# Sawyerbatch/simglucose

Measured on AMD Instinct MI355X. Metric: env-steps/sec at batch=1M patients (1-min dt); fp64 glucose trace max-abs-err, higher is better.
Workload: dtype f64

## Files before the change

simglucose_amd/csrc/t1d_abi.hip:

```cpp
#include "../../include/t1d.h"
#include "t1d_kernels.hpp"
#include "t1d_dopri5.hpp"
#include "t1d_policy.hpp"

#include <climits>
#include <cmath>
#include <cstdio>
#include <cstring>
#include <new>
#include <string>
#include <vector>

using namespace t1d;

struct t1d_ctx {
    int device = -1;
    int np = 0, S = 0;
    double sensor[T1D_SENSOR_NCOLS];
    double pump[T1D_PUMP_NCOLS];
    double* d_par64 = nullptr; float* d_par32 = nullptr;
    double* d_raw64 = nullptr;
    double* d_x0 = nullptr;
    double* d_minv64 = nullptr; float* d_minv32 = nullptr;
    int* d_status = nullptr;
    int math = 1;
    int n_cu = 256;
    int lds_per_block = 65536;
    std::vector<std::pair<const void*, size_t>> lds_allowed;
    int s1_blocks = 0;
    int split_refill = 1;
    int adaptive_gut = 1;
    int single_minute_kernel = 1;
    int integrator = -1;
    int split_nsub = 0;
    int np_pad = 0;
    double* d_prop64 = nullptr; float* d_prop32 = nullptr;
    long long* d_trace = nullptr;
    int defer_min_chunks = 1;
    int multi_minute_kernel = 1;
    int multi_minute_min_envs = 262144, multi_minute_min_envs_f32 = 393216;
    int park_cap = 0;
    int pingpong = 1;
    mutable unsigned launches = 0;
    int record_group_min = 64;
    int rollout_launches = 1;
    int rollout_launches_min_envs = 524288, rollout_launches_min_envs_f32 = 786432;
    int restart_compact = 1;
    std::vector<double> ptab;
    std::vector<double> dpar;
};

static thread_local std::string g_err;
static int fail(int code, const std::string& msg) { g_err = msg; return code; }
#define T1D_HIP(call)                                                                         \
    do {                                                                                      \
        hipError_t _e = (call);                                                               \
        if (_e != hipSuccess)                                                                 \
            return fail(T1D_E_HIP, std::string(#call) + ": " + hipGetErrorString(_e));        \
    } while (0)

static std::vector<double> spline_second_derivative_operator()
{
    const int K = 11;
    const double h = 15.0;
    std::vector<double> A(K * K, 0.0), B(K * K, 0.0);
    for (int k = 1; k < K - 1; ++k) {
        A[k * K + k - 1] = 1.0; A[k * K + k] = 4.0; A[k * K + k + 1] = 1.0;
        B[k * K + k - 1] = 6.0 / (h * h); B[k * K + k] = -12.0 / (h * h); B[k * K + k + 1] = 6.0 / (h * h);
    }
    A[0] = 1.0; A[1] = -2.0; A[2] = 1.0;
    A[(K - 1) * K + K - 3] = 1.0; A[(K - 1) * K + K - 2] = -2.0; A[(K - 1) * K + K - 1] = 1.0;
    for (int c = 0; c < K; ++c) {
        int piv = c;
        for (int r = c + 1; r < K; ++r) if (std::fabs(A[r * K + c]) > std::fabs(A[piv * K + c])) piv = r;
        if (piv != c) for (int j = 0; j < K; ++j) { std::swap(A[c * K + j], A[piv * K + j]); std::swap(B[c * K + j], B[piv * K + j]); }
        const double d = A[c * K + c];
        for (int j = 0; j < K; ++j) { A[c * K + j] /= d; B[c * K + j] /= d; }
        for (int r = 0; r < K; ++r) {
            if (r == c) continue;
            const double f = A[r * K + c];
            if (f == 0.0) continue;
            for (int j = 0; j < K; ++j) { A[r * K + j] -= f * A[c * K + j]; B[r * K + j] -= f * B[c * K + j]; }
        }
    }
    return B;
}


static void mat_expm(int n, const double* A, double* E)
{
    double nrm = 0.0;
    for (int i = 0; i < n; ++i) { double r = 0.0; for (int j = 0; j < n; ++j) r += std::fabs(A[i * n + j]); nrm = std::max(nrm, r); }
    int sq = 0;
    while (nrm > 0.03125 && sq < 60) { nrm *= 0.5; ++sq; }
    const double sc = std::ldexp(1.0, -sq);
    std::vector<double> B(n * n), term(n * n, 0.0), tmp(n * n);
    for (int k = 0; k < n * n; ++k) B[k] = A[k] * sc;
    for (int i = 0; i < n; ++i) { for (int j = 0; j < n; ++j) E[i * n + j] = (i == j); term[i * n + i] = 1.0; }
    for (int d = 1; d <= 16; ++d) {
        for (int i = 0; i < n; ++i)
            for (int j = 0; j < n; ++j) {
                double v = 0.0;
                for (int k = 0; k < n; ++k) v += term[i * n + k] * B[k * n + j];
                tmp[i * n + j] = v / (double)d;
            }
        term = tmp;
        for (int k = 0; k < n * n; ++k) E[k] += term[k];
    }
    for (int q = 0; q < sq; ++q) {
        for (int i = 0; i < n; ++i)
            for (int j = 0; j < n; ++j) {
                double v = 0.0;
                for (int k = 0; k < n; ++k) v += E[i * n + k] * E[k * n + j];
                tmp[i * n + j] = v;
            }
        for (int k = 0; k < n * n; ++k) E[k] = tmp[k];
    }
}

// ... 9 lines not shown
    at(5, 5) = -r[T1D_P_KI]; at(5, 0) = r[T1D_P_KI] / r[T1D_P_VI];
    at(6, 6) = -r[T1D_P_KI]; at(6, 5) = r[T1D_P_KI];
    double Ah[81], Ph[81], Pk[81], tmp[81];
    const int nb = 2 * n_sub;
    const double hb = 1.0 / (double)nb;
    for (int k = 0; k < 81; ++k) Ah[k] = A[k] * hb;
    mat_expm(9, Ah, Ph);
    std::memcpy(Pk, Ph, sizeof(Pk));
    static const int c6[7] = {4, 0, 1, 2, 3, 7, 8};
    static const int c8[7] = {6, 5, 0, 1, 2, 3, 7};
    for (int k = 1; k <= nb; ++k) {
        double* o = out + (k - 1) * 14;
        for (int j = 0; j < 7; ++j) { o[j] = Pk[4 * 9 + c6[j]]; o[7 + j] = Pk[6 * 9 + c8[j]]; }
        if (k == nb) break;
        for (int i = 0; i < 9; ++i)
            for (int j = 0; j < 9; ++j) {
                double v = 0.0;
                for (int q = 0; q < 9; ++q) v += Ph[i * 9 + q] * Pk[q * 9 + j];
                tmp[i * 9 + j] = v;
            }
        std::memcpy(Pk, tmp, sizeof(Pk));
    }
    double* t = out + 14 * nb;
    static const int c5[5] = {0, 1, 2, 3, 7};
    for (int j = 0; j < 5; ++j) { t[j] = Pk[0 * 9 + c5[j]]; t[5 + j] = Pk[1 * 9 + c5[j]]; }
    t[10] = Pk[2 * 9 + 2]; t[11] = Pk[2 * 9 + 7];
    t[12] = Pk[3 * 9 + 2]; t[13] = Pk[3 * 9 + 3]; t[14] = Pk[3 * 9 + 7];
    static const int c7[6] = {5, 0, 1, 2, 3, 7};
    for (int j = 0; j < 6; ++j) t[15 + j] = Pk[5 * 9 + c7[j]];
    const double h1 = 1.0 / (double)n_sub;
    const double hs[2] = {h1, 0.5 * h1};
    for (int part = 0; part < 2; ++part) {
        const double hh = hs[part], z = r[T1D_P_KABS] * hh;
        double I[3];
        for (int k = 0; k < 3; ++k) {
            double term = 1.0, sum = 0.0;
            for (int q = 1; q <= k + 1; ++q) term /= (double)q;
            for (int q = 1; q <= k; ++q) term *= (double)q;
            for (int j = 0; j < 60; ++j) {
                sum += term;
                term *= -z / (double)(k + j + 2);
                if (std::fabs(term) < 1e-30) break;
            }
            I[k] = sum;
        }
        double* w = out + kPropRows(n_sub) + 4 * part;
        w[0] = std::exp(-z);
        w[1] = hh * (2.0 * I[2] - 3.0 * I[1] + I[0]);
        w[2] = hh * (-4.0 * I[2] + 4.0 * I[1]);
        w[3] = hh * (2.0 * I[2] - I[1]);
    }
}

extern "C" int t1d_split_tables(const double* patient_row, int n_cols, int n_sub, double* out, int out_len)
{
    if (!patient_row || !out) return fail(T1D_E_INVALID, "t1d_split_tables: NULL argument");
    if (n_cols != T1D_P_NCOLS) return fail(T1D_E_INVALID, "t1d_split_tables: n_cols must be T1D_P_NCOLS (45)");
    if (n_sub < 2 || n_sub > 8 || (n_sub & 1)) return fail(T1D_E_INVALID, "t1d_split_tables: n_sub must be 2, 4, 6 or 8");
    if (out_len < kPropRows(n_sub) + 8) return fail(T1D_E_INVALID, "t1d_split_tables: out_len < 28 n_sub + 29");
    split_tables_row(patient_row, n_sub, out);
    return T1D_OK;
}

static int ensure_split(t1d_ctx* c, int ng)
{
    static_assert(DP_X2WB2 == DP_X2E + 7 && DP_X2E2 == DP_X2E + 4, "x2 weight rows are consecutive");
    if (c->split_nsub == ng) return T1D_OK;
    T1D_HIP(hipDeviceSynchronize());
    const int rows = kPropRows(ng), npp = c->np_pad;
    std::vector<double> prop((size_t)rows * npp, 0.0), one((size_t)rows + 8);
    for (int j = 0; j < c->np; ++j) {
        split_tables_row(c->ptab.data() + (size_t)j * T1D_P_NCOLS, ng, one.data());
        for (int k = 0; k < rows; ++k) prop[(size_t)k * npp + j] = one[k];
        for (int k = 0; k < 8; ++k) c->dpar[(size_t)(DP_X2E + k) * kMaxPatients + j] = one[rows + k];
    }
    std::vector<float> propf(prop.begin(), prop.end()), dpf(c->dpar.begin(), c->dpar.end());
    (void)hipFree(c->d_prop64); (void)hipFree(c->d_prop32); c->d_prop64 = nullptr; c->d_prop32 = nullptr;
    T1D_HIP(hipMalloc((void**)&c->d_prop64, prop.size() * 8));
    T1D_HIP(hipMalloc((void**)&c->d_prop32, propf.size() * 4));
    T1D_HIP(hipMemcpy(c->d_prop64, prop.data(), prop.size() * 8, hipMemcpyHostToDevice));
    T1D_HIP(hipMemcpy(c->d_prop32, propf.data(), propf.size() * 4, hipMemcpyHostToDevice));
    T1D_HIP(hipMemcpy(c->d_par64, c->dpar.data(), c->dpar.size() * 8, hipMemcpyHostToDevice));
    T1D_HIP(hipMemcpy(c->d_par32, dpf.data(), dpf.size() * 4, hipMemcpyHostToDevice));
    c->split_nsub = ng;
    return T1D_OK;
}

#if T1D_S1_TRACE
extern "C" int t1d_debug_trace(t1d_ctx* c, long long* out) { return hipMemcpy(out, c->d_trace, 128 * 4 * 64 * sizeof(long long), hipMemcpyDeviceToHost) == hipSuccess ? 0 : -1; }
#endif
extern "C" int t1d_abi_version(void) { return T1D_ABI_VERSION; }
extern "C" const char* t1d_last_error(void) { return g_err.c_str(); }

extern "C" int t1d_ctx_create(int hip_device, const double* ptab, int n_patients, int n_cols,
                              const double* sensor_row, const double* pump_row, t1d_ctx** out)
{
    try {
        if (!out) return fail(T1D_E_INVALID, "t1d_ctx_create: out is NULL");
        *out = nullptr;
        if (!ptab || !sensor_row || !pump_row) return fail(T1D_E_INVALID, "t1d_ctx_create: NULL table");
        if (n_cols != T1D_P_NCOLS) return fail(T1D_E_INVALID, "t1d_ctx_create: n_cols must be T1D_P_NCOLS (45)");
        if (n_patients < 1 || n_patients > kMaxPatients)
            return fail(T1D_E_INVALID, "t1d_ctx_create: n_patients must be in [1, 64]");
        const double st = sensor_row[5];
        if (!(st >= 1.0) || st != std::floor(st) || st > 1440.0)
            return fail(T1D_E_INVALID, "t1d_ctx_create: sensor sample_time must be a whole number of minutes >= 1");
        if (st > 150.0) return fail(T1D_E_INVALID, "t1d_ctx_create: sensor sample_time must be <= 150 minutes");
        for (int k = 2; k < 6; k += 3)
            if (!(pump_row[k] > 0.0)) return fail(T1D_E_INVALID, "t1d_ctx_create: pump increments must be > 0");
        int ndev = 0;
        if (hipGetDeviceCount(&ndev) != hipSuccess || ndev < 1)
            return fail(T1D_E_NODEVICE, "t1d_ctx_create: no HIP device visible");
        if (hip_device < 0 || hip_device >= ndev) return fail(T1D_E_INVALID, "t1d_ctx_create: bad device index");
        T1D_HIP(hipSetDevice(hip_device));
        int n_cu = 0;
        T1D_HIP(hipDeviceGetAttribute(&n_cu, hipDeviceAttributeMultiprocessorCount, hip_device));

        t1d_ctx* c = new (std::nothrow) t1d_ctx();
        if (!c) return fail(T1D_E_INVALID, "t1d_ctx_create: out of host memory");
        int lds_max = 0;
        if (hipDeviceGetAttribute(&lds_max, hipDeviceAttributeMaxSharedMemoryPerBlock, hip_device) == hipSuccess && lds_max > 0) c->lds_per_block = lds_max;
        c->device = hip_device; c->n_cu = n_cu > 0 ? n_cu : 256; c->np = n_patients; c->S = (int)std::floor(150.0 / st);
        std::memcpy(c->sensor, sensor_row, sizeof(c->sensor));
        std::memcpy(c->pump, pump_row, sizeof(c->pump));

        const int np = n_patients;
        std::vector<double> dp((size_t)DP_COUNT * kMaxPatients, 0.0), x0((size_t)13 * np);
        for (int j = 0; j < np; ++j) {
            const double* r = ptab + (size_t)j * n_cols;
            auto set = [&](int idx, double v) { dp[(size_t)idx * kMaxPatients + j] = v; };
            set(DP_KMAX, r[T1D_P_KMAX]); set(DP_KMIN, r[T1D_P_KMIN]); set(DP_KABS, r[T1D_P_KABS]);
            set(DP_HK, (r[T1D_P_KMAX] - r[T1D_P_KMIN]) / 2.0);
            set(DP_B, r[T1D_P_B]); set(DP_D, r[T1D_P_D]);
            set(DP_CAA, 5.0 / 2.0 / (1.0 - r[T1D_P_B])); set(DP_CCC, 5.0 / 2.0 / r[T1D_P_D]);
            set(DP_RATC, r[T1D_P_F] * r[T1D_P_KABS] / r[T1D_P_BW]);
            set(DP_KP1, r[T1D_P_KP1]); set(DP_KP2, r[T1D_P_KP2]); set(DP_KP3, r[T1D_P_KP3]);
            set(DP_FSNC, r[T1D_P_FSNC]); set(DP_KE1, r[T1D_P_KE1]); set(DP_KE2, r[T1D_P_KE2]);
            set(DP_K1, r[T1D_P_K1]); set(DP_K2, r[T1D_P_K2]); set(DP_VM0, r[T1D_P_VM0]);
            set(DP_VMX, r[T1D_P_VMX]); set(DP_KM0, r[T1D_P_KM0]);
            set(DP_M24, r[T1D_P_M2] + r[T1D_P_M4]); set(DP_M1, r[T1D_P_M1]);
            set(DP_KA1, r[T1D_P_KA1]); set(DP_KA2, r[T1D_P_KA2]); set(DP_VI, r[T1D_P_VI]);
            set(DP_P2U, r[T1D_P_P2U]); set(DP_IB, r[T1D_P_IB]); set(DP_KI, r[T1D_P_KI]);
            set(DP_M130, r[T1D_P_M1] + r[T1D_P_M30]); set(DP_M2, r[T1D_P_M2]);
            set(DP_KA1KD, r[T1D_P_KA1] + r[T1D_P_KD]); set(DP_KD, r[T1D_P_KD]); set(DP_KSC, r[T1D_P_KSC]);
            set(DP_INSC, 6000.0 / r[T1D_P_BW]); set(DP_VG, r[T1D_P_VG]); set(DP_IVI, 1.0 / r[T1D_P_VI]); set(DP_IVG, 1.0 / r[T1D_P_VG]);
            set(DP_DK, r[T1D_P_KMAX] - r[T1D_P_KMIN]);
            set(DP_CF, r[T1D_P_F] / r[T1D_P_BW]);
            for (int k = 0; k < 13; ++k) x0[(size_t)k * np + j] = r[T1D_P_X0 + k];
        }
        std::vector<double> raw((size_t)kRawPars * kMaxPatients, 0.0);
        for (int j = 0; j < np; ++j)
            for (int k = 0; k < kRawPars; ++k) raw[(size_t)k * kMaxPatients + j] = ptab[(size_t)j * n_cols + T1D_P_BW + k];
        c->ptab.assign(ptab, ptab + (size_t)np * n_cols);
        c->dpar = dp;
        c->np_pad = (np + 1) & ~1;
        std::vector<float> dpf(dp.begin(), dp.end());
        const std::vector<double> minv = spline_second_derivative_operator();
        std::vector<float> minvf(minv.begin(), minv.end());
        auto up = [&](void** dst, const void* src, size_t bytes) -> hipError_t {
            hipError_t e = hipMalloc(dst, bytes);
            if (e != hipSuccess) return e;
            return hipMemcpy(*dst, src, bytes, hipMemcpyHostToDevice);
        };
        hipError_t e = hipSuccess;
        if (e == hipSuccess) e = up((void**)&c->d_par64, dp.data(), dp.size() * 8);
        if (e == hipSuccess) e = up((void**)&c->d_par32, dpf.data(), dpf.size() * 4);
        if (e == hipSuccess) e = up((void**)&c->d_x0, x0.data(), x0.size() * 8);
        if (e == hipSuccess) e = up((void**)&c->d_raw64, raw.data(), raw.size() * 8);
        if (e == hipSuccess) e = up((void**)&c->d_minv64, minv.data(), minv.size() * 8);
        if (e == hipSuccess) e = up((void**)&c->d_minv32, minvf.data(), minvf.size() * 4);
#if T1D_S1_TRACE
        if (e == hipSuccess) e = hipMalloc((void**)&c->d_trace, 128 * 4 * 64 * sizeof(long long));
        if (e == hipSuccess) e = hipMemset(c->d_trace, 0, 128 * 4 * 64 * sizeof(long long));
#endif
        if (e == hipSuccess) e = hipMalloc((void**)&c->d_status, sizeof(int));
        if (e == hipSuccess) e = hipMemset(c->d_status, 0, sizeof(int));
        if (e != hipSuccess) {
            std::string m = std::string("t1d_ctx_create: ") + hipGetErrorString(e);
            t1d_ctx_destroy(c);
            return fail(T1D_E_HIP, m);
        }
        *out = c;
        return T1D_OK;
    } catch (const std::exception& ex) {
        return fail(T1D_E_INVALID, std::string("t1d_ctx_create: ") + ex.what());
    } catch (...) {
        return fail(T1D_E_INVALID, "t1d_ctx_create: unknown exception");
    }
}

extern "C" int t1d_ctx_set_option(t1d_ctx* c, const char* name, int64_t value)
{
    if (!c || !name) return fail(T1D_E_INVALID, "t1d_ctx_set_option: NULL argument");
    struct Opt { const char* name; int t1d_ctx::*field; int64_t lo, hi; };
    static const Opt opts[] = {
        {"math", &t1d_ctx::math, 0, 1},
        {"split_refill", &t1d_ctx::split_refill, 0, 1},
        {"defer_min_chunks", &t1d_ctx::defer_min_chunks, 0, 65535},
        {"multi_minute_kernel", &t1d_ctx::multi_minute_kernel, 0, 2},
        {"multi_minute_min_envs", &t1d_ctx::multi_minute_min_envs, 0, 1 << 28},
        {"multi_minute_min_envs_f32", &t1d_ctx::multi_minute_min_envs_f32, 0, 1 << 28},
        {"park_cap", &t1d_ctx::park_cap, 0, 65535},
        {"pingpong", &t1d_ctx::pingpong, 0, 1},
        {"record_group_min", &t1d_ctx::record_group_min, 1, 64},
        {"rollout_launches", &t1d_ctx::rollout_launches, 0, 2},
        {"rollout_launches_min_envs", &t1d_ctx::rollout_launches_min_envs, 0, 1 << 28},
        {"rollout_launches_min_envs_f32", &t1d_ctx::rollout_launches_min_envs_f32, 0, 1 << 28},
        {"restart_compact", &t1d_ctx::restart_compact, 0, 1},
        {"s1_blocks", &t1d_ctx::s1_blocks, 0, 65535},
        {"adaptive_gut", &t1d_ctx::adaptive_gut, 0, 3},
        {"single_minute_kernel", &t1d_ctx::single_minute_kernel, 0, 1},
        {"integrator", &t1d_ctx::integrator, -1, 1},
    };
    for (const Opt& o : opts)
        if (std::strcmp(name, o.name) == 0) {
            if (value < o.lo || value > o.hi)
                return fail(T1D_E_INVALID, std::string("t1d_ctx_set_option: ") + name + " must be in [" + std::to_string(o.lo) + ", " + std::to_string(o.hi) + "]");
            c->*(o.field) = (int)value;
            return T1D_OK;
        }
    return fail(T1D_E_INVALID, std::string("t1d_ctx_set_option: unknown option ") + name);
}

extern "C" int t1d_ctx_destroy(t1d_ctx* c)
{
    if (!c) return T1D_OK;
    (void)hipSetDevice(c->device);
    (void)hipFree(c->d_par64); (void)hipFree(c->d_par32); (void)hipFree(c->d_x0);
    (void)hipFree(c->d_minv64); (void)hipFree(c->d_minv32); (void)hipFree(c->d_status);
    (void)hipFree(c->d_prop64); (void)hipFree(c->d_prop32); (void)hipFree(c->d_trace); (void)hipFree(c->d_raw64);
    delete c;
    return T1D_OK;
}

static int check_batch(const char* who, const t1d_ctx* c, const t1d_batch* b, bool need_action)
{
    if (!c) return fail(T1D_E_INVALID, std::string(who) + ": ctx is NULL");
    if (!b) return fail(T1D_E_INVALID, std::string(who) + ": batch is NULL");
    if (b->n < 1 || b->n > (int64_t)1 << 28)
        return fail(T1D_E_INVALID, std::string(who) + ": batch.n out of range");
    if (b->dtype != T1D_F64 && b->dtype != T1D_F32) return fail(T1D_E_INVALID, std::string(who) + ": bad dtype");
    if (!b->x || !b->planned || !b->last_qsto || !b->last_food || !b->t || !b->meta || !b->last_cgm ||
        !b->ar_e || !b->pts || !b->prev_risk)
        return fail(T1D_E_INVALID, std::string(who) + ": a state pointer is NULL");
    if (!b->cgm || !b->bg || !b->reward || !b->done)
        return fail(T1D_E_INVALID, std::string(who) + ": cgm/bg/reward/done outputs are required");
    if (need_action && !b->basal) return fail(T1D_E_INVALID, std::string(who) + ": basal is NULL");
    if (b->n_meals < 0 || b->n_meals > 65535) return fail(T1D_E_INVALID, std::string(who) + ": n_meals out of range");
    if (b->n_meals > 0 && (!b->meal_time || !b->meal_amt))
        return fail(T1D_E_INVALID, std::string(who) + ": n_meals > 0 but meal table pointer is NULL");
    if (b->n_normals < 0) return fail(T1D_E_INVALID, std::string(who) + ": n_normals < 0");
    if (b->n_normals > 0 && !b->normals) return fail(T1D_E_INVALID, std::string(who) + ": n_normals > 0 but normals is NULL");
    const int known = T1D_BATCH_NO_PUMP | T1D_BATCH_NO_REFILL_DUE | (T1D_AB_FLAGS ? 0x1f00 : 0);
    if (b->flags & ~known) return fail(T1D_E_INVALID, std::string(who) + ": unknown bit in batch.flags");
    if (hipSetDevice(c->device) != hipSuccess) return fail(T1D_E_HIP, std::string(who) + ": hipSetDevice failed");
    return T1D_OK;
}

template <typename T>
static KArgs<T> make_args(const t1d_ctx* c, const t1d_batch* b, int minutes, int n_sub)
{
    KArgs<T> a;
    a.n = b->n; a.env_offset = b->env_offset; a.seed = b->seed;
    a.x = (T*)b->x; a.planned = (T*)b->planned; a.last_qsto = (T*)b->last_qsto; a.last_food = (T*)b->last_food;
    a.t = b->t; a.meta = b->meta; a.episode = b->episode; a.next_meal = b->next_meal;
    a.last_cgm = (T*)b->last_cgm; a.ar_e = (T*)b->ar_e; a.pts = (T*)b->pts; a.prev_risk = (T*)b->prev_risk; a.dbar = (T*)b->dbar;
    a.basal = (const T*)b->basal; a.bolus = (const T*)b->bolus; a.cho = (const T*)b->cho;
    a.meal_time = b->meal_time; a.meal_amt = (const T*)b->meal_amt;
    a.normals = b->n_normals > 0 ? (const T*)b->normals : nullptr;
    a.x0_override = (const T*)b->x0_override;
    a.cgm = (T*)b->cgm; a.bg = (T*)b->bg; a.reward = (T*)b->reward; a.done = b->done;
    a.lbgi = (T*)b->lbgi; a.hbgi = (T*)b->hbgi; a.risk = (T*)b->risk; a.meal = (T*)b->meal; a.insulin = (T*)b->insulin; a.cgm0 = (T*)b->cgm0;
    a.dpar = sizeof(T) == 8 ? (const T*)c->d_par64 : (const T*)c->d_par32;
    a.x0tab = c->d_x0;
    a.minv = sizeof(T) == 8 ? (const T*)c->d_minv64 : (const T*)c->d_minv32;
    a.status = c->d_status; a.trace = c->d_trace;
    a.sen.pacf = (T)c->sensor[0]; a.sen.gamma = (T)c->sensor[1]; a.sen.lambda = (T)c->sensor[2];
    a.sen.delta = (T)c->sensor[3]; a.sen.xi = (T)c->sensor[4]; a.sen.st = (int)c->sensor[5];
    a.sen.vmin = (T)c->sensor[6]; a.sen.vmax = (T)c->sensor[7];
    a.pump.min_bolus = (T)c->pump[0]; a.pump.max_bolus = (T)c->pump[1]; a.pump.inc_bolus = (T)c->pump[2];
    a.pump.min_basal = (T)c->pump[3]; a.pump.max_basal = (T)c->pump[4]; a.pump.inc_basal = (T)c->pump[5];
    a.np = c->np; a.S = c->S; a.n_meals = b->n_meals; a.n_normals = b->n_normals;
    a.minutes = minutes; a.n_sub = n_sub; a.flags = b->flags | (c->pingpong && (c->launches & 1) ? kFlagReverse : 0);
    a.prop = sizeof(T) == 8 ? (const T*)c->d_prop64 : (const T*)c->d_prop32;
    a.prop_rows = c->split_nsub ? kPropRows(c->split_nsub) : 0; a.np_pad = c->np_pad;
    return a;
}

static inline dim3 grid_for(int64_t n) { return dim3((unsigned)((n + kBlock - 1) / kBlock)); }

extern "C" int t1d_reset(t1d_ctx* c, const t1d_batch* b, const uint8_t* mask, int random_init_bg, void* stream)
{
    int rc = check_batch("t1d_reset", c, b, false);
    if (rc) return rc;
    hipStream_t s = (hipStream_t)stream;
    if (b->dtype == T1D_F64)
        hipLaunchKernelGGL(reset_kernel<double>, grid_for(b->n), dim3(kBlock), 0, s, make_args<double>(c, b, 1, 1), mask, random_init_bg);
    else
        hipLaunchKernelGGL(reset_kernel<float>, grid_for(b->n), dim3(kBlock), 0, s, make_args<float>(c, b, 1, 1), mask, random_init_bg);
    T1D_HIP(hipGetLastError());
    return T1D_OK;
}

static hipError_t allow_lds(t1d_ctx* c, const void* fn, size_t bytes)
{
    if (bytes <= 65536) return hipSuccess;
    for (auto& f : c->lds_allowed)
        if (f.first == fn) {
            if (f.second >= bytes) return hipSuccess;
            hipError_t e = hipFuncSetAttribute(fn, hipFuncAttributeMaxDynamicSharedMemorySize, (int)bytes);
            if (e == hipSuccess) f.second = bytes;
            return e;
        }
    hipError_t e = hipFuncSetAttribute(fn, hipFuncAttributeMaxDynamicSharedMemorySize, (int)bytes);
    if (e == hipSuccess) c->lds_allowed.push_back({fn, bytes});
    return e;
}

enum class Kern { step, rollout, step1, step1d, stepn };

struct Plan {
    Kern kernel = Kern::step;
    bool f64 = true;
    int variant = 0;
    bool refill = false;
    int stride = 32;
    bool extra = false;
    bool tiered = false;
    bool ctrl = false;
    bool refill_ahead = false;
    bool tables = false;
    unsigned grid = 0, block = 0;
    size_t lds = 0;
    int nchunks = 0, cap = 0, mode = 0;
};

static bool is_packed(const t1d_batch* b, size_t esz)
{
    const char* xb = (const char*)b->x;
    const size_t rowb = (size_t)b->n * esz;
    return (const char*)b->planned == xb + 13 * rowb && (const char*)b->last_qsto == xb + 14 * rowb &&
           (const char*)b->last_food == xb + 15 * rowb && (const char*)b->last_cgm == xb + 16 * rowb &&
           (const char*)b->prev_risk == xb + 17 * rowb && (const char*)b->pts == xb + 18 * rowb &&
           (const char*)b->dbar == xb + (size_t)kRowDbar * rowb &&
           b->next_meal && (const char*)b->meta == (const char*)b->t + (size_t)b->n * 4 &&
           (const char*)b->next_meal == (const char*)b->t + (size_t)b->n * 8 &&
           (size_t)kPackedRows * rowb < ((size_t)1 << 32);
}

static int plan_call(const char* who, const t1d_ctx* c, const t1d_batch* b, int minutes, int n_sub, bool rollout, Plan* out,
                     bool one_launch = false)
{
    Plan& p = *out;
    p = Plan();
    if (minutes < 1 || minutes > 100000) return fail(T1D_E_INVALID, std::string(who) + ": minutes out of range");
    if (n_sub < 1 || n_sub > 4096) return fail(T1D_E_INVALID, std::string(who) + ": n_sub out of range");
    bool split = c->math != 0 && n_sub >= 2 && n_sub <= 8 && !(n_sub & 1);
    if (c->integrator == 1 && !split)
        return fail(T1D_E_INVALID, std::string(who) + ": the split integrator needs math = 1 and n_sub in {2, 4, 6, 8}");
    split = split && c->integrator != 0;
    p.tables = split;
    p.f64 = b->dtype == T1D_F64;
    const size_t esz = p.f64 ? 8 : 4;
    p.extra = b->lbgi || b->hbgi || b->risk || b->meal || b->insulin;
    const bool split_refill = c->math != 0 && c->split_refill && minutes <= (int)c->sensor[5];

    const int stride = c->np <= 32 ? 32 : 64;
// ... 519 lines not shown
```

simglucose_amd/csrc/t1d_device.hpp:

```cpp
#pragma once
#include <hip/hip_runtime.h>
#include <rocrand/rocrand_kernel.h>
#include <stdint.h>

namespace t1d {

enum DevPar : int {
    DP_KMAX = 0, DP_KMIN, DP_KABS, DP_HK , DP_B, DP_D, DP_CAA ,
    DP_CCC , DP_RATC , DP_KP1, DP_KP2, DP_KP3, DP_FSNC, DP_KE1, DP_KE2,
    DP_K1, DP_K2, DP_VM0, DP_VMX, DP_KM0, DP_M24 , DP_M1, DP_KA1, DP_KA2, DP_VI, DP_P2U,
    DP_IB, DP_KI, DP_M130 , DP_M2, DP_KA1KD , DP_KD, DP_KSC, DP_INSC ,
    DP_VG, DP_IVI , DP_IVG , DP_DK ,
    DP_CF , DP_X2E , DP_X2WA, DP_X2WM, DP_X2WB,
    DP_X2E2, DP_X2WA2, DP_X2WM2, DP_X2WB2, DP_COUNT
};
constexpr int DP_RK4_COUNT = DP_CF;
constexpr int kMaxPatients = 64;
constexpr int kBlock = 256;

template <typename T> struct ParsLds {
    static constexpr bool kSplitRk4 = false;
    const T* base;
    int pid;
    __device__ __forceinline__ T operator()(int idx) const { return base[idx * kMaxPatients + pid]; }
// ... 496 lines not shown
__device__ __forceinline__ void rk4_minute(P& p, const MinuteIn<T>& u, T (&x)[13], int n_sub)
{
    if (MATH == 1 && P::kSplitRk4) {
        rk4_substeps_split(p, u, x, n_sub);
    } else {
        rk4_substeps<MATH>(p, u, x, n_sub);
    }
}

template <int MATH, typename T, typename P>
__device__ __forceinline__ void rk4_substeps(P& p, const MinuteIn<T>& u, T (&x)[13], int n_sub)
{
    const T h = T(1) / T(n_sub);
    const T hh = T(0.5) * h, h6 = h / T(6);
    T k[13], y[13], acc[13];
    for (int s = 0; s < n_sub; ++s) {
        rhs<MATH>(p, u, x, k);
#pragma unroll
        for (int i = 0; i < 13; ++i) { acc[i] = k[i]; y[i] = x[i] + hh * k[i]; }
        rhs<MATH>(p, u, y, k);
#pragma unroll
        for (int i = 0; i < 13; ++i) { acc[i] += T(2) * k[i]; y[i] = x[i] + hh * k[i]; }
        rhs<MATH>(p, u, y, k);
#pragma unroll
        for (int i = 0; i < 13; ++i) { acc[i] += T(2) * k[i]; y[i] = x[i] + h * k[i]; }
        rhs<MATH>(p, u, y, k);
#pragma unroll
        for (int i = 0; i < 13; ++i) x[i] = x[i] + h6 * (acc[i] + k[i]);
    }
}

__device__ __forceinline__ double dbar_of(double lq, double lf) { return fma(lf, 1000.0, lq); }
__device__ __forceinline__ float dbar_of(float lq, float lf) { return fmaf(lf, 1000.0f, lq); }

template <int MATH, typename T, typename P>
__device__ __forceinline__ MinuteIn<T> eat_minute(P& p, const T (&x)[13], T meal, T insulin_upm,
                                                  T& planned, T& last_qsto, T& last_food, bool& was_eating)
{
    T to_eat = T(0);
    planned += meal;
    if (planned > T(0)) {
        to_eat = planned < T(5) ? planned : T(5);
        planned -= to_eat;
        planned = planned > T(0) ? planned : T(0);
    }
    if (to_eat > T(0) && !was_eating) {
        last_qsto = x[0] + x[1];
        last_food = T(0);
    }
    last_food += to_eat;
    was_eating = to_eat > T(0);
    MinuteIn<T> u;
    u.d_mg = to_eat * T(1000);
    u.ins = insulin_upm * p(DP_INSC);
    const T dbar = dbar_of(last_qsto, last_food);
    u.has_dbar = dbar > T(0);
    const T dsafe = u.has_dbar ? dbar : T(1);
    if (MATH == 0) {
        u.aa = u.has_dbar ? p(DP_CAA) / dsafe : T(0);
        u.cc = u.has_dbar ? p(DP_CCC) / dsafe : T(0);
    } else {
        const T inv2 = u.has_dbar ? fdiv(T(2), dsafe) : T(0);
        u.aa = p(DP_CAA) * inv2;
        u.cc = p(DP_CCC) * inv2;
    }
    u.bD = p(DP_B) * dsafe;
    u.dD = p(DP_D) * dsafe;
    u.aabD = u.aa * u.bD;
    u.ccdD = u.cc * u.dD;
    return u;
}

template <typename T>
__device__ __forceinline__ T pump_quantise(T amount, T inc, T lo, T hi)
{
    T v = amount * T(6000);
    v = t_rint(v / inc) * inc;
    v = fdiv(v, T(6000));
    v = v < hi ? v : hi;
    v = v > lo ? v : lo;
    return v;
}

template <int MATH, typename T>
__device__ __forceinline__ void risk_index1(T bg, T& lbgi, T& hbgi, T& ri)
{
    T f;
    if (MATH == 0) {
        f = T(1.509) * (t_pow(t_log(bg), T(1.084)) - T(5.381));
    } else {
        const T inf = T(__builtin_huge_val());
        const T nan = T(__builtin_nan(""));
        const bool regular = bg > T(1) && bg < inf;
        const T u = log_core<true>(regular ? bg : T(2));
        const T pw = exp_core<12, true>(T(1.084) * log_core<true>(u));
        const T freg = T(1.509) * (pw - T(5.381));
        const T fodd = bg == T(1) ? T(1.509) * (T(0) - T(5.381)) : ((bg == T(0) || bg == inf) ? inf : nan);
        f = regular ? freg : fodd;
    }
    T l = T(0), h = T(0);
    const T ff = T(10) * f * f;
    l = f < T(0) ? ff : T(0);
    h = f > T(0) ? ff : T(0);
    const T big = sizeof(T) == 8 ? T(1.7976931348623157e308) : T(3.4028234663852886e38);
    l = l < big ? l : big;
    h = h < big ? h : big;
    lbgi = l; hbgi = h; ri = l + h;
}

template <typename T> struct SensorC { T pacf, gamma, lambda, delta, xi, vmin, vmax; int st; };
template <typename T> struct PumpC { T min_bolus, max_bolus, inc_bolus, min_basal, max_basal, inc_basal; };

template <bool FAST, typename T>
__device__ __forceinline__ T johnson_su(const SensorC<T>& s, T e)
{
    const T v = (e - s.gamma) / s.delta;
    if (!FAST) return s.xi + s.lambda * t_sinh(v);
    const T lim = sizeof(T) == 8 ? T(350) : T(40);
    const T E = exp_core(t_max(t_min(v, lim), -lim));
    return s.xi + s.lambda * (T(0.5) * (E - fdiv(T(1), E)));
}

__device__ __forceinline__ double2 philox_pair(uint64_t seed, uint64_t gid, uint32_t episode, uint32_t pair)
{
    rocrand_state_philox4x32_10 st;
    const unsigned long long off = 4ull * (((unsigned long long)episode << 24) + pair);
    rocrand_init(seed, gid, off, &st);
    return rocrand_normal_double2(&st);
}

}
```

simglucose_amd/csrc/t1d_kernels.hpp:

```cpp
#pragma once
#include "../../include/t1d.h"
#include "t1d_device.hpp"

#ifndef T1D_WAVES
#define T1D_WAVES 2
#endif
#ifndef T1D_ROW_RECOMPUTE
#define T1D_ROW_RECOMPUTE 1
#endif
constexpr int kFlagReverse = 0x10000;
#ifndef T1D_AB_FLAGS
#define T1D_AB_FLAGS 0
#endif

#include <climits>
#include <cstdint>
#include <type_traits>

namespace t1d {

template <typename T> struct KArgs {
    int64_t n, env_offset;
    uint64_t seed;
    T* x; T* planned; T* last_qsto; T* last_food; int32_t* t; uint32_t* meta; uint32_t* episode; int32_t* next_meal;
    T* last_cgm; T* ar_e; T* pts; T* prev_risk; T* dbar;
    const T* basal; const T* bolus; const T* cho; const int32_t* meal_time; const T* meal_amt;
    const T* normals; const T* x0_override;
    T* cgm; T* bg; T* reward; uint8_t* done; T* lbgi; T* hbgi; T* risk; T* meal; T* insulin; T* cgm0;
    const T* dpar;
    const T* prop;
    const double* x0tab;
    const T* minv;
    int* status;
    long long* trace;
    SensorC<T> sen; PumpC<T> pump;
    int np, S, n_meals, n_normals, minutes, n_sub, flags, prop_rows, np_pad;
};

template <typename T> struct PidArgs {
    T P, I, D, target;
    T* integ; T* prev; T* sum_risk; T* min_bg; T* max_bg; int32_t* n_low; int32_t* n_high;
    int n_steps;
    int kind;
    const T* bb_basal; const T* bb_cr; const T* bb_cf; T* bb_prev_meal;
    T* bg_trace; T* cgm_trace; T* cho_trace; T* ins_trace; int64_t trace_row;
};

template <typename U> __device__ __forceinline__ U* row(U* base, int64_t n, int k)
{
#if T1D_ROW_RECOMPUTE
    int kk = k;
    asm volatile("" : "+s"(kk));
    return base + (int64_t)kk * n;
#else
    U* p = base + (int64_t)k * n;
    asm volatile("" : "+s"(p));
    return p;
#endif
}
template <typename U> __device__ __forceinline__ U* rowv(U* base, int64_t n, int k) { return base + (int64_t)k * n; }
template <typename A> __device__ __forceinline__ bool ab_flag(const A& a, int bit) { return T1D_AB_FLAGS && (a.flags & bit) != 0; }
template <typename U> struct GRef {
    __attribute__((address_space(1))) U* p;
    __device__ __forceinline__ operator U() const { return *p; }
    __device__ __forceinline__ const GRef& operator=(U v) const { *p = v; return *this; }
};
template <typename U> __device__ __forceinline__ GRef<U> at(U* base, unsigned i)
{
    typedef __attribute__((address_space(1))) char gchar;
    typedef __attribute__((address_space(1))) U gU;
    return GRef<U>{(gU*)((gchar*)base + (unsigned)(i * (unsigned)sizeof(U)))};
}

typedef unsigned int t1d_v2u32 __attribute__((ext_vector_type(2)));
template <typename U> struct BRow { __amdgpu_buffer_rsrc_t r; int soff; };
template <typename U> struct BRef {
    __amdgpu_buffer_rsrc_t r; unsigned voff; int soff;
    __device__ __forceinline__ operator U() const
    {
        if constexpr (sizeof(U) == 8) return __builtin_bit_cast(U, __builtin_amdgcn_raw_buffer_load_b64(r, voff, soff, 0));
        else return __builtin_bit_cast(U, __builtin_amdgcn_raw_buffer_load_b32(r, voff, soff, 0));
    }
    __device__ __forceinline__ const BRef& operator=(U v) const
    {
        if constexpr (sizeof(U) == 8) __builtin_amdgcn_raw_buffer_store_b64(__builtin_bit_cast(t1d_v2u32, v), r, voff, soff, 0);
        else __builtin_amdgcn_raw_buffer_store_b32(__builtin_bit_cast(unsigned, v), r, voff, soff, 0);
        return *this;
    }
};
template <typename U> struct BRows {
    __amdgpu_buffer_rsrc_t r; int rowbytes;
    __device__ __forceinline__ BRows(U* base, int64_t n, int rows)
        : r(__builtin_amdgcn_make_buffer_rsrc(base, 0, (int)(rows * n * (int64_t)sizeof(U)), 0x00020000)), rowbytes((int)(n * (int64_t)sizeof(U))) {}
    __device__ __forceinline__ BRow<U> operator()(int k) const { return BRow<U>{r, k * rowbytes}; }
};
template <typename U> __device__ __forceinline__ BRef<U> at(BRow<U> row, unsigned i) { return BRef<U>{row.r, (unsigned)(i * (unsigned)sizeof(U)), row.soff}; }

template <typename T> struct Env {
    T x[13];
    T planned, lq, lf, last_cgm, prev_risk;
    T cur[4];
    int t, cursor, next_meal, next_meal_loaded;
    bool eating;
};
template <typename T> struct StepOut { T cgm, bg, meal, ins; };

template <typename T>
__device__ __forceinline__ void stage_pars(const KArgs<T>& a, T* lds, int rows = DP_COUNT)
{
    const int tot = rows * kMaxPatients;
    for (int j = threadIdx.x; j < tot; j += blockDim.x) lds[j] = a.dpar[j];
    __syncthreads();
}
// ... 376 lines not shown
    if (a.flags & T1D_BATCH_NO_PUMP) {
        q_basal = basal; q_bolus = a.bolus ? bolus : T(0);
    } else {
        int z = 0;
        asm volatile("" : "+v"(z));
        const T* lc = lconst + z;
        q_basal = pump_quantise(basal, lc[0], lc[1], lc[2]);
        q_bolus = lc[4] > T(0) ? lc[4] : T(0);
        if (a.bolus) q_bolus = pump_quantise(bolus, lc[3], lc[4], lc[5]);
    }
    const T insulin = q_basal + q_bolus;
    T meal;
    if (a.cho) {
        meal = at(a.cho, i);
        asm volatile("" : "+v"(meal));
    } else {
        meal = meal_lookup<T, true>(a, i, e);
    }
    ParsLdsS<T, STRIDE> pl{ldp, (int)pid};
    MinuteIn<T> u = eat_minute<1, T>(pl, e.x, meal, insulin, e.planned, e.lq, e.lf, e.eating);
    T f1 = T(0);
    if (MODE == 2) {
        const TierPre<T> tp = tier_pre(pl, u, e.x);
        f1 = tp.f1;
        on_level(tp.level2);
        if (tp.level2) return;
    }
    {
        const bool live0 = (meta & (T1D_META_EATING | T1D_META_PLANNED)) != 0 || (T1D_AB_FLAGS && (a.flags & 0x1000));
        const bool changed = live0 ? (e.planned != planned0 || e.lq != lq0 || e.lf != lf0) : (e.eating || e.planned > T(0));
        if (changed) {
            at(X(13), i) = e.planned; at(X(14), i) = e.lq; at(X(15), i) = e.lf;
            at(X(kRowDbar), i) = dbar_of(e.lq, e.lf);
        }
    }
    at(I(0), i) = e.t + 1;
    if (e.next_meal != e.next_meal_loaded) at(I(2), i) = e.next_meal;
    {
        const uint32_t meta1 = pid | (e.eating ? T1D_META_EATING : 0u) | (e.planned > T(0) ? T1D_META_PLANNED : 0u) | ((uint32_t)e.cursor << 16);
        if (meta1 != meta) at(I(1), i) = (int32_t)meta1;
    }
    if (EXTRA) {
        if (a.meal) at(a.meal, i) = meal;
        if (a.insulin) at(a.insulin, i) = insulin;
    }
    S1_MARK(2);
#if T1D_S1_PHASE_PRIO
    if (MODE != 3) __builtin_amdgcn_s_setprio(0);
#endif
    if (!ab_flag(a, 0x800)) {
        PropLdsS<T, STRIDE> pr{lpr, (int)pid};
        if (MODE == 1) {
            split_minute_tiered(pl, pr, u, e.x, a.n_sub);
        } else if (REG) {
            ParsReg<T> p;
#pragma unroll
            for (int k = 0; k < (int)(sizeof(kSplitPars) / sizeof(int)); ++k) p.v[kSplitPars[k]] = pl(kSplitPars[k]);
#pragma unroll
            for (int k = 0; k < 4; ++k) p.v[kSplitW(LEVEL) + k] = pl(kSplitW(LEVEL) + k);
            p.pin_split();
            split_level<LEVEL, T, ParsReg<T>, decltype(pr), MODE == 2>(p, pr, u, e.x, a.n_sub, f1);
        } else {
            split_level<LEVEL, T, ParsLdsS<T, STRIDE>, decltype(pr), MODE == 2>(pl, pr, u, e.x, a.n_sub, f1);
        }
    }
    S1_MARK(3);
#if T1D_S1_PHASE_PRIO
    __builtin_amdgcn_s_setprio(T1D_S1_PHASE_PRIO);
#endif
#pragma unroll
    for (int k = 0; k < 13; ++k) at(X(k), i) = e.x[k];
#pragma unroll
    for (int k = 0; k < 4; ++k) e.cur[k] = at(X(40 + k), i);
    T last_cgm = a.sen.st == 1 ? T(0) : (T)at(X(16), i);
    const T rp = at(X(17), i);
    S1_MARK(4);
    bool due, entered = false;
    const T noise = measure_noise<false>(a, i, e, due, &entered);
    if (entered) {
#pragma unroll
        for (int k = 0; k < 4; ++k) at(X(40 + k), i) = e.cur[k];
    }
    const T gsub = e.x[12] * pl(DP_IVG);
    if (due) {
        T c = gsub + noise;
        int z = 0;
        asm volatile("" : "+v"(z));
        const T vmin = lconst[6 + z], vmax = lconst[7 + z];
        c = c > vmin ? c : vmin;
        c = c < vmax ? c : vmax;
        last_cgm = c;
        if (a.sen.st != 1) at(X(16), i) = c;
    }
    const T cgm_out = last_cgm, bg_out = gsub;
    at(a.cgm, i) = cgm_out; at(a.bg, i) = bg_out;
    if (!(fabs((double)e.x[12]) <= 1.0e300)) atomicOr(a.status, T1D_ST_NONFINITE);
    T l, h, r, rc = T(0);
    if (!ab_flag(a, 0x100)) risk_index1<1>(cgm_out, l, h, rc);
    at(a.reward, i) = rp - rc;
    at(X(17), i) = rc;
    at(a.done, i) = (bg_out < T(70) || bg_out > T(350)) ? 1 : 0;
    if (EXTRA && (a.lbgi || a.hbgi || a.risk)) {
        risk_index1<1>(bg_out, l, h, r);
        if (a.lbgi) at(a.lbgi, i) = l;
        if (a.hbgi) at(a.hbgi, i) = h;
        if (a.risk) at(a.risk, i) = r;
    }
#if T1D_S1_TRACE
    if (tr && (threadIdx.x & 63) == 0 && tk < 6) tr[tk * 8 + 5] = (long long)wall_clock64();
#endif
    S1_MARK(6);
}

struct S1NoLevel { __device__ __forceinline__ void operator()(bool) const {} };

template <typename T, int STRIDE>
__device__ __forceinline__ void s1_stage_tables(const KArgs<T>& a, T* ldp, T* lpr, T* lconst)
{
    for (int j = threadIdx.x; j < DP_COUNT * STRIDE; j += (int)blockDim.x) {
        const int r = j / STRIDE, c = j % STRIDE;
        ldp[j] = c < a.np ? a.dpar[r * kMaxPatients + c] : T(0);
    }
    for (int j = threadIdx.x; j < a.prop_rows * STRIDE; j += (int)blockDim.x) {
        const int r = j / STRIDE, c = j % STRIDE;
        lpr[j] = c < a.np ? a.prop[r * a.np_pad + c] : T(0);
    }
    if (threadIdx.x == 0) {
        lconst[0] = a.pump.inc_basal; lconst[1] = a.pump.min_basal; lconst[2] = a.pump.max_basal;
        lconst[3] = a.pump.inc_bolus; lconst[4] = a.pump.min_bolus; lconst[5] = a.pump.max_bolus;
        lconst[6] = a.sen.vmin; lconst[7] = a.sen.vmax;
    }
}

template <typename T, int STRIDE, bool EXTRA, bool TIERED>
__global__ __launch_bounds__(s1_threads<T>(), 1) void step1_kernel(const KArgs<T> a, int nchunks)
{
    T* const ldp = (T*)t1d_dyn_lds;
    T* const lpr = ldp + DP_COUNT * STRIDE;
    __shared__ int queue;
    __shared__ T lconst[8];
    s1_stage_tables<T, STRIDE>(a, ldp, lpr, lconst);
    if (threadIdx.x == 0) queue = 0;
    __syncthreads();
    const int per_block = (nchunks + (int)gridDim.x - 1) / (int)gridDim.x;
    const int first = (int)blockIdx.x * per_block;
    const int count = nchunks - first < per_block ? nchunks - first : per_block;
    const unsigned lane = threadIdx.x & 63u;
#if T1D_S1_TRACE
    long long* tr = (a.trace && blockIdx.x < 32) ? a.trace + (blockIdx.x * (s1_threads<T>() / 64) + threadIdx.x / 64) * 64 : nullptr;
#else
    long long* tr = nullptr;
#endif
    int tk = -1;
    for (int it = 0;; ++it) {
        int c = 0;
        if (lane == 0) c = atomicAdd(&queue, 1);
        c = __builtin_amdgcn_readfirstlane(c);
        if (c >= count) break;
        const unsigned i = (unsigned)(first + c) * 64u + lane;
        __builtin_assume(i < (1u << 28));
        ++tk;
        if ((int64_t)i < a.n) s1_chunk<!TIERED, T, STRIDE, EXTRA, TIERED ? 1 : 0>(a, ldp, lpr, lconst, i, s1_load(a, i), S1NoLevel(), tr, tk);
    }
}

template <typename T, bool EXTRA>
__global__ __launch_bounds__(s1d_threads<T>(), 1) void step1d_kernel(const KArgs<T> a, int nchunks)
{
    constexpr int STRIDE = 32;
    T* const ldp = (T*)t1d_dyn_lds;
    T* const lpr = ldp + DP_COUNT * STRIDE;
    const int per_block = (nchunks + (int)gridDim.x - 1) / (int)gridDim.x;
    const unsigned lane = threadIdx.x & 63u;
    T* const park_t = lpr + a.prop_rows * STRIDE;
    int* const park_i = (int*)(park_t + 18 * kS1DPark);
    uint16_t* const list = (uint16_t*)(park_i + 3 * kS1DPark);
    __shared__ int queue, taken, listed, passed;
    __shared__ T lconst[8];
    s1_stage_tables<T, STRIDE>(a, ldp, lpr, lconst);
    if (threadIdx.x == 0) { queue = 0; taken = 0; listed = 0; passed = 0; }
    __syncthreads();
    const int first = (int)blockIdx.x * per_block;
    const int count = nchunks - first < per_block ? nchunks - first : per_block;
    const unsigned base = (unsigned)first * 64u;
    long long* tr = nullptr;
#if T1D_S1_TRACE
    long long* const ph = (a.trace && blockIdx.x < 32) ? a.trace + (blockIdx.x * (s1d_threads<T>() / 64) + threadIdx.x / 64) * 64 : nullptr;
#define S1D_PHASE(k) do { if (ph && lane == 0) ph[k] = (long long)wall_clock64(); } while (0)
#else
#define S1D_PHASE(k) do { } while (0)
#endif
    S1D_PHASE(0);
    auto draw = [&](int* counter) -> int {
        int g = 0;
        if (lane == 0) g = atomicAdd(counter, 1);
        return __builtin_amdgcn_readfirstlane(g);
    };
    auto on_level = [&](unsigned i, const S1In<T>& in) {
        return [&, i](bool level2) {
            if (level2) {
                const int slot = atomicAdd(&listed, 1);
                list[slot] = (uint16_t)(i - base);
                if (slot < kS1DPark) s1_park(in, park_t, park_i, slot);
            }
            __builtin_amdgcn_fence(__ATOMIC_RELEASE, "workgroup");
            if (lane == 0) atomicAdd(&passed, 1);
        };
    };
    int it = 0;
    for (;; ++it) {
        const int c = draw(&queue);
        if (c >= count) break;
        const unsigned i = (unsigned)(first + ((a.flags & kFlagReverse) ? count - 1 - c : c)) * 64u + lane;
        __builtin_assume(i < (1u << 28));
        if ((int64_t)i < a.n) {
#if T1D_S1_TRACE
            tr = ph ? ph + 16 : nullptr;
#endif
            const S1In<T> in = s1_load(a, i);
            s1_chunk<true, T, STRIDE, EXTRA, 2>(a, ldp, lpr, lconst, i, in, on_level(i, in), tr, it);
        }
    }
    tr = nullptr;
    S1D_PHASE(1);
    while (__hip_atomic_load(&passed, __ATOMIC_RELAXED, __HIP_MEMORY_SCOPE_WORKGROUP) < count) __builtin_amdgcn_s_sleep(4);
    __builtin_amdgcn_fence(__ATOMIC_ACQUIRE, "workgroup");
    __builtin_amdgcn_s_setprio(3);
    const int total = __hip_atomic_load(&listed, __ATOMIC_RELAXED, __HIP_MEMORY_SCOPE_WORKGROUP);
    S1D_PHASE(2);
#if T1D_S1_TRACE
    if (ph && lane == 0) { ph[6] = total; ph[7] = 0; ph[8] = it; }
#endif
    for (;;) {
        const int lo = draw(&taken) * 64;
        if (lo >= total) break;
        if (lo + (int)lane < total) {
            const unsigned i = base + (unsigned)list[lo + (int)lane];
            __builtin_assume(i < (1u << 28));
            const S1In<T> in = lo + 64 <= kS1DPark ? s1_unpark<T>(park_t, park_i, lo + (int)lane) : s1_load(a, i);
            s1_chunk<true, T, STRIDE, EXTRA, 3>(a, ldp, lpr, lconst, i, in, S1NoLevel(), nullptr, 0);
        }
    }
    __builtin_amdgcn_s_waitcnt(0x0070);
    S1D_PHASE(3);
    S1D_PHASE(4);
#undef S1D_PHASE
}

template <typename T> struct SnLane {
    T x[13];
    T planned, lq, lf, insulin, bg_sum, cgm_sum, meal_sum, last_cgm;
    int t, next_meal, cursor, m;
    unsigned i;
    uint32_t pid;
    int dirty;
    bool eating;
};
constexpr int kSnParkT = 21, kSnParkI = 5;
constexpr int kSnDirtyShift = 9;
constexpr int kSnConst = 20;
constexpr int kSnSpinLimit = 1 << 20;

// ... 830 lines not shown
```

Baseline: 12.64 billion.

## Stage prebuilt LDS table image with vector copies; fast-path clamped risk index

Builds a host-side packed image of the parameter and propagation tables plus pump and sensor constants, laid out at stride 32, and copies it into LDS with 16-byte vector loads. This replaces the per-element strided staging with div/mod indexing in the step kernels. It also adds a wave-uniform fast path for the risk index: when the CGM clamp bounds guarantee a positive, finite value, it uses the unchecked log/exp cores. The image is only built when np<=32. The STRIDE==32 kernels now assume the image exists, so a null image would break them if they were ever used with more patients.

```diff
diff --git a/simglucose_amd/csrc/t1d_abi.hip b/simglucose_amd/csrc/t1d_abi.hip
--- a/simglucose_amd/csrc/t1d_abi.hip
+++ b/simglucose_amd/csrc/t1d_abi.hip
@@ -35,6 +35,7 @@
     int split_nsub = 0;
     int np_pad = 0;
     double* d_prop64 = nullptr; float* d_prop32 = nullptr;
+    double* d_img64 = nullptr; float* d_img32 = nullptr;
     long long* d_trace = nullptr;
     int defer_min_chunks = 1;
     int multi_minute_kernel = 1;
@@ -210,6 +211,23 @@
     T1D_HIP(hipMemcpy(c->d_prop32, propf.data(), propf.size() * 4, hipMemcpyHostToDevice));
     T1D_HIP(hipMemcpy(c->d_par64, c->dpar.data(), c->dpar.size() * 8, hipMemcpyHostToDevice));
     T1D_HIP(hipMemcpy(c->d_par32, dpf.data(), dpf.size() * 4, hipMemcpyHostToDevice));
+    (void)hipFree(c->d_img64); (void)hipFree(c->d_img32); c->d_img64 = nullptr; c->d_img32 = nullptr;
+    if (c->np <= 32) {
+        std::vector<double> img((size_t)(DP_COUNT + rows) * 32 + kImgConst, 0.0);
+        for (int j = 0; j < c->np; ++j) {
+            for (int k = 0; k < DP_COUNT; ++k) img[(size_t)k * 32 + j] = c->dpar[(size_t)k * kMaxPatients + j];
+            for (int k = 0; k < rows; ++k) img[(size_t)(DP_COUNT + k) * 32 + j] = prop[(size_t)k * npp + j];
+        }
+        double* const lc = img.data() + (size_t)(DP_COUNT + rows) * 32;
+        lc[0] = c->pump[5]; lc[1] = c->pump[3]; lc[2] = c->pump[4];
+        lc[3] = c->pump[2]; lc[4] = c->pump[0]; lc[5] = c->pump[1];
+        lc[6] = c->sensor[6]; lc[7] = c->sensor[7];
+        std::vector<float> imgf(img.begin(), img.end());
+        T1D_HIP(hipMalloc((void**)&c->d_img64, img.size() * 8));
+        T1D_HIP(hipMalloc((void**)&c->d_img32, imgf.size() * 4));
+        T1D_HIP(hipMemcpy(c->d_img64, img.data(), img.size() * 8, hipMemcpyHostToDevice));
+        T1D_HIP(hipMemcpy(c->d_img32, imgf.data(), imgf.size() * 4, hipMemcpyHostToDevice));
+    }
     c->split_nsub = ng;
     return T1D_OK;
 }
@@ -357,6 +375,7 @@
     (void)hipFree(c->d_par64); (void)hipFree(c->d_par32); (void)hipFree(c->d_x0);
     (void)hipFree(c->d_minv64); (void)hipFree(c->d_minv32); (void)hipFree(c->d_status);
     (void)hipFree(c->d_prop64); (void)hipFree(c->d_prop32); (void)hipFree(c->d_trace); (void)hipFree(c->d_raw64);
+    (void)hipFree(c->d_img64); (void)hipFree(c->d_img32);
     delete c;
     return T1D_OK;
 }
@@ -411,6 +430,7 @@
     a.np = c->np; a.S = c->S; a.n_meals = b->n_meals; a.n_normals = b->n_normals;
     a.minutes = minutes; a.n_sub = n_sub; a.flags = b->flags | (c->pingpong && (c->launches & 1) ? kFlagReverse : 0);
     a.prop = sizeof(T) == 8 ? (const T*)c->d_prop64 : (const T*)c->d_prop32;
+    a.img = sizeof(T) == 8 ? (const T*)c->d_img64 : (const T*)c->d_img32;
     a.prop_rows = c->split_nsub ? kPropRows(c->split_nsub) : 0; a.np_pad = c->np_pad;
     return a;
 }
diff --git a/simglucose_amd/csrc/t1d_device.hpp b/simglucose_amd/csrc/t1d_device.hpp
--- a/simglucose_amd/csrc/t1d_device.hpp
+++ b/simglucose_amd/csrc/t1d_device.hpp
@@ -602,10 +602,20 @@
     return v;
 }
 
-template <int MATH, typename T>
+template <int MATH, typename T, bool CLAMPED = false>
 __device__ __forceinline__ void risk_index1(T bg, T& lbgi, T& hbgi, T& ri)
 {
     T f;
+    if (MATH == 1 && CLAMPED) {
+        const T u = log_core<true>(bg);
+        const T pw = exp_core<12, true>(T(1.084) * log_core<true>(u));
+        f = T(1.509) * (pw - T(5.381));
+        const T ff = T(10) * f * f;
+        lbgi = f < T(0) ? ff : T(0);
+        hbgi = f > T(0) ? ff : T(0);
+        ri = ff;
+        return;
+    }
     if (MATH == 0) {
         f = T(1.509) * (t_pow(t_log(bg), T(1.084)) - T(5.381));
     } else {
diff --git a/simglucose_amd/csrc/t1d_kernels.hpp b/simglucose_amd/csrc/t1d_kernels.hpp
--- a/simglucose_amd/csrc/t1d_kernels.hpp
+++ b/simglucose_amd/csrc/t1d_kernels.hpp
@@ -29,6 +29,7 @@
     T* cgm; T* bg; T* reward; uint8_t* done; T* lbgi; T* hbgi; T* risk; T* meal; T* insulin; T* cgm0;
     const T* dpar;
     const T* prop;
+    const T* img;
     const double* x0tab;
     const T* minv;
     int* status;
@@ -571,11 +572,13 @@
         for (int k = 0; k < 4; ++k) at(X(40 + k), i) = e.cur[k];
     }
     const T gsub = e.x[12] * pl(DP_IVG);
+    bool in_range = false;
     if (due) {
         T c = gsub + noise;
         int z = 0;
         asm volatile("" : "+v"(z));
         const T vmin = lconst[6 + z], vmax = lconst[7 + z];
+        in_range = vmin > T(1) && vmax < T(__builtin_huge_val());
         c = c > vmin ? c : vmin;
         c = c < vmax ? c : vmax;
         last_cgm = c;
@@ -585,7 +588,10 @@
     at(a.cgm, i) = cgm_out; at(a.bg, i) = bg_out;
     if (!(fabs((double)e.x[12]) <= 1.0e300)) atomicOr(a.status, T1D_ST_NONFINITE);
     T l, h, r, rc = T(0);
-    if (!ab_flag(a, 0x100)) risk_index1<1>(cgm_out, l, h, rc);
+    if (!ab_flag(a, 0x100)) {
+        if (__builtin_amdgcn_ballot_w64(!in_range) == 0ull) risk_index1<1, T, true>(cgm_out, l, h, rc);
+        else risk_index1<1>(cgm_out, l, h, rc);
+    }
     at(a.reward, i) = rp - rc;
     at(X(17), i) = rc;
     at(a.done, i) = (bg_out < T(70) || bg_out > T(350)) ? 1 : 0;
@@ -603,6 +609,31 @@
 
 struct S1NoLevel { __device__ __forceinline__ void operator()(bool) const {} };
 
+constexpr int kImgConst = 8;
+template <typename T, int NT>
+__device__ __forceinline__ void s1_stage_image(const KArgs<T>& a, T* ldp, T* lconst)
+{
+    typedef unsigned int u32x4 __attribute__((ext_vector_type(4)));
+    const int words = (DP_COUNT + a.prop_rows) * 32;
+    const int units = words * (int)sizeof(T) / 16;
+    const u32x4* __restrict__ src = (const u32x4*)a.img;
+    u32x4* dst = (u32x4*)ldp;
+    for (int j0 = 0; j0 < units; j0 += 4 * NT) {
+        u32x4 v[4];
+#pragma unroll
+        for (int k = 0; k < 4; ++k) {
+            const int j = j0 + k * NT + (int)threadIdx.x;
+            v[k] = j < units ? src[j] : u32x4{0u, 0u, 0u, 0u};
+        }
+#pragma unroll
+        for (int k = 0; k < 4; ++k) {
+            const int j = j0 + k * NT + (int)threadIdx.x;
+            if (j < units) dst[j] = v[k];
+        }
+    }
+    if (threadIdx.x < kImgConst) lconst[threadIdx.x] = a.img[words + threadIdx.x];
+}
+
 template <typename T, int STRIDE>
 __device__ __forceinline__ void s1_stage_tables(const KArgs<T>& a, T* ldp, T* lpr, T* lconst)
 {
@@ -628,7 +659,8 @@
     T* const lpr = ldp + DP_COUNT * STRIDE;
     __shared__ int queue;
     __shared__ T lconst[8];
-    s1_stage_tables<T, STRIDE>(a, ldp, lpr, lconst);
+    if constexpr (STRIDE == 32) s1_stage_image<T, s1_threads<T>()>(a, ldp, lconst);
+    else s1_stage_tables<T, STRIDE>(a, ldp, lpr, lconst);
     if (threadIdx.x == 0) queue = 0;
     __syncthreads();
     const int per_block = (nchunks + (int)gridDim.x - 1) / (int)gridDim.x;
@@ -666,7 +698,7 @@
     uint16_t* const list = (uint16_t*)(park_i + 3 * kS1DPark);
     __shared__ int queue, taken, listed, passed;
     __shared__ T lconst[8];
-    s1_stage_tables<T, STRIDE>(a, ldp, lpr, lconst);
+    s1_stage_image<T, s1d_threads<T>()>(a, ldp, lconst);
     if (threadIdx.x == 0) { queue = 0; taken = 0; listed = 0; passed = 0; }
     __syncthreads();
     const int first = (int)blockIdx.x * per_block;
```

Measured after the change: 12.87 billion (median of 6 runs). 1.02x the previous value.
